# tychedelia/josefine

Measured on NVIDIA H100. Metric: Raft-group ticks/sec @ 64Ki groups x 5 replicas, higher is better.
Workload: dtype u64

## Files before the change

josefine_b200/csrc/sym_fold.cuh:

```cuda
#pragma once
#include "raft_device.cuh"

namespace jr {
#ifdef JR_DEVICE_CODE

struct SymMail {
  uint32_t hb, hb_commit;
  uint32_t ae, ae_nb, ae_id[JR_MAX_AE_BLOCKS];
  uint32_t mk;
  uint32_t hbr, hbr_commit, hbr_has;
  uint32_t ar, ar_head;
  __device__ __forceinline__ uint32_t id(uint32_t k) const {
    uint32_t v = ae_id[0];
#pragma unroll
    for (uint32_t j = 1; j < JR_MAX_AE_BLOCKS; ++j)
      if (k == j) v = ae_id[j];
    return v;
  }
  __device__ __forceinline__ void set_id(uint32_t k, uint32_t v) {
#pragma unroll
    for (uint32_t j = 0; j < JR_MAX_AE_BLOCKS; ++j)
      if (k == j) ae_id[j] = v;
  }
};

constexpr uint32_t SYM_ROWS = 8;
#ifndef JR_SYM_LANES
#define JR_SYM_LANES 128
#endif
constexpr uint32_t SYM_LANES = JR_SYM_LANES;
constexpr uint32_t SYM_ENC_L = 5, SYM_ENC_F = 3;
constexpr uint32_t SYM_SMEM_UNITS = 2 * SYM_ROWS + SYM_ENC_L + SYM_ENC_F;
constexpr uint32_t SYM2_GROUPS = 64;
constexpr uint32_t SYM2_UNITS = SYM_SMEM_UNITS + 2 * 2 + 2 * 1;
constexpr uint32_t SYM2_ABORT = 1u << 8, SYM2_IDS = 1u << 9, SYM2_MODE = 1u << 10;
enum : uint32_t {
  SP_MAIL_IN = 0,
  SP_AR = 1,
  SP_CLIENT = 2,
  SP_ENC_NOTIFY = 3,
  SP_ENC_APPLY = 4,
  SP_MAIL_OUT = 5,
  SP_BARRIER = 6,
  SP_HB = 7,
  SP_SCAN = 8,
  SP_EXTEND = 9,
  SP_ENTER = 10, SP_FILL = 11, SP_LEAVE = 12, SP_TRUNC = 13,
};

template <int R, bool SPLIT = false>
struct SymGroup {
  static constexpr uint32_t STRIDE = SPLIT ? SYM2_GROUPS : SYM_LANES;
  const Dev& d;
  const uint32_t g;
  const size_t plane;
  uint32_t L;
  uint32_t F0;
  uint64_t term, hbtime, now;
  uint32_t head, commit, idgen, maxkey, ckey, ph_self, mode_self, ph_f, mode_f;
  uint32_t fhead, fcommit, fmaxkey, fckey;
  uint32_t n_hb;
  uint64_t last_hb;
  uint32_t tbase;
  uint32_t flo;
  uint4* rows;
  uint4* enc;
  uint32_t lcnt, fcnt;
  uint32_t lwend, fwend;
  uint32_t n_app;
  bool abort;
  bool share;
#ifdef JR_PROFILE
  long long pt;
  uint32_t prole, pslot;
  __device__ __forceinline__ uint32_t phase(uint32_t slot) {
    const uint32_t o = pslot;
    if constexpr (SPLIT) {
      JR_PROF_ADD(prole, o, pt);
      pslot = slot;
    }
    return o;
  }
#else
  __device__ __forceinline__ uint32_t phase(uint32_t) const { return 0; }
#endif

  __device__ __forceinline__ SymGroup(const Dev& dv, uint32_t g_) : d(dv), g(g_), plane((size_t)R * dv.Gp) {
#ifdef JR_PROFILE
    pt = 0; prole = JR_ROLE_CANDIDATE; pslot = 0;
#endif
  }
  __device__ __forceinline__ size_t rg(uint32_t r) const { return (size_t)r * d.Gp + g; }
  __device__ __forceinline__ size_t row(uint32_t r, uint32_t bid) const { return (size_t)(bid & d.capm) * plane + rg(r); }
  __device__ __forceinline__ bool in_window(uint32_t bid) const { return bid - tbase < d.cap; }
  __device__ __forceinline__ uint4& slot(uint32_t r, uint32_t bid) const { return rows[((r == L ? 0u : SYM_ROWS) + (bid % SYM_ROWS)) * STRIDE]; }
  __device__ __forceinline__ void cache_put(uint32_t r, uint32_t bid, uint32_t nx, uint64_t tk) const {
    slot(r, bid) = make_uint4(bid, nx, (uint32_t)tk, (uint32_t)(tk >> 32));
  }
  __device__ __forceinline__ void fetch(uint32_t r, uint32_t bid, uint32_t& next, uint64_t& tok) {
    if (!in_window(bid)) { next = ABSENT; tok = 0; return; }
    const uint4 e = slot(r, bid);
    if (e.x == bid) { next = e.y; tok = (uint64_t)e.z | ((uint64_t)e.w << 32); return; }
    next = __ldcg(d.cnext + row(r, bid));
    tok = __ldcg(d.ctok + row(r, bid));
    if (!SPLIT) cache_put(r, bid, next, tok);
  }
  __device__ __forceinline__ void fetch_sent(uint32_t bid, uint32_t mk_sent, uint32_t n_app, uint32_t& next, uint64_t& tok) {
    if (!SPLIT) { fetch(L, bid, next, tok); return; }
    if (!in_window(bid)) { next = ABSENT; tok = 0; return; }
    if (bid + SYM_ROWS > mk_sent + n_app) {
      const uint4 e = slot(L, bid);
      if (e.x == bid) { next = e.y; tok = (uint64_t)e.z | ((uint64_t)e.w << 32); return; }
    }
    next = __ldcg(d.cnext + row(L, bid));
    tok = __ldcg(d.ctok + row(L, bid));
  }
  __device__ __forceinline__ void cache_clear(uint32_t first = 0, uint32_t n = 2 * SYM_ROWS) const {
#pragma unroll
    for (uint32_t k = 0; k < 2 * SYM_ROWS; ++k)
      if (k >= first && k < first + n) rows[k * STRIDE] = make_uint4(ABSENT, ABSENT, 0u, 0u);
  }
  __device__ __forceinline__ void cache_fill(uint32_t r, uint32_t top) const {
    uint32_t nx[SYM_ROWS];
    uint64_t tk[SYM_ROWS];
#pragma unroll
    for (uint32_t j = 0; j < SYM_ROWS; ++j)
      if (j <= top && in_window(top - j)) {
        nx[j] = d.cnext[row(r, top - j)];
        tk[j] = d.ctok[row(r, top - j)];
      }
#pragma unroll
    for (uint32_t j = 0; j < SYM_ROWS; ++j)
      if (j <= top && in_window(top - j)) cache_put(r, top - j, nx[j], tk[j]);
  }
  __device__ __forceinline__ bool has(uint32_t r, uint32_t bid) {
    uint32_t n; uint64_t t;
    fetch(r, bid, n, t);
    return n != ABSENT;
  }
  __device__ __forceinline__ void fetch_f(uint32_t bid, uint32_t& next, uint64_t& tok) {
    if (in_window(bid) && bid < flo) { abort = true; next = ABSENT; tok = 0; return; }
    fetch(F0, bid, next, tok);
  }
  __device__ __forceinline__ bool has_f(uint32_t bid) {
    uint32_t n; uint64_t t;
    fetch_f(bid, n, t);
    return n != ABSENT;
  }

  __device__ __forceinline__ uint4& eq(uint32_t k) const { return enc[k * STRIDE]; }
  __device__ __forceinline__ FsmOut leader_out() const { return FsmOut{d.fs + rg(L), plane, d.F, g, L}; }
  __device__ __forceinline__ FsmOut followers_out() const {
    return FsmOut{d.fs + rg(F0), plane, d.F, g, F0, ((1u << R) - 1u) & ~(1u << L)};
  }
  __device__ __forceinline__ void enc_init_leader(uint2 leader_fc) {
    eq(0) = make_uint4(leader_fc.x, leader_fc.y, leader_fc.y, 0u);
#pragma unroll
    for (uint32_t k = 1; k < SYM_ENC_L; ++k) eq(k) = make_uint4(0u, 0u, 0u, 0u);
    lwend = FS_PATTERN_BITS;
  }
  __device__ __forceinline__ void enc_init_followers() {
#pragma unroll
    for (uint32_t k = SYM_ENC_L; k < SYM_ENC_L + SYM_ENC_F; ++k) eq(k) = make_uint4(0u, 0u, 0u, 0u);
    fwend = FS_PATTERN_BITS;
  }
  template <bool NOTIFY>
  __device__ __forceinline__ bool run_extend(uint4& q, uint2& qs, uint32_t bid, uint32_t nxa, uint64_t tok) const {
    const uint4 r = q;
    if (!r.y || bid != r.x || r.y >= FS_MAX_RUN || nxa != (NOTIFY ? FSR_CLIENT : bid - 1u)) return false;
    const uint2 st = qs;
    const uint64_t step = tok - ((uint64_t)r.z | ((uint64_t)r.w << 32));
    if (r.y == 1u) {
      if (st.x != (NOTIFY ? FSR_CLIENT : bid - 2u)) return false;
      qs = make_uint2((uint32_t)step, (uint32_t)(step >> 32));
    } else if (step != ((uint64_t)st.x | ((uint64_t)st.y << 32))) {
      return false;
    }
    q = make_uint4(bid + 1u, r.y + 1u, (uint32_t)tok, (uint32_t)(tok >> 32));
    return true;
  }
  template <bool NOTIFY>
  __device__ __forceinline__ void emit_leader(uint32_t bid, uint32_t nxa, uint64_t tok) {
    if (!(d.flags & JR_F_CAPTURE_FSM)) return;
    if (lcnt >= d.Fr) { abort = true; return; }
    const uint32_t outer = phase(NOTIFY ? SP_ENC_NOTIFY : SP_ENC_APPLY);
    if (lcnt + 1u != lwend &&
        run_extend<NOTIFY>(eq(NOTIFY ? 4 : 2), reinterpret_cast<uint2*>(&eq(3))[NOTIFY ? 1 : 0], bid, nxa, tok)) {
      if (NOTIFY) {
        const uint32_t b = lcnt + FS_PATTERN_BITS - lwend;
        uint32_t* w = b < 128u ? reinterpret_cast<uint32_t*>(&eq(1)) + (b >> 5) : &eq(0).w;
        *w |= 1u << (b & 31u);
      }
      ++lcnt;
      phase(outer);
      return;
    }
    FsmEnc e;
    const uint4 q0 = eq(0);
    e.nrec = q0.x; e.seq = q0.y + lcnt; e.wseq = q0.z; e.pb2 = q0.w;
    ++lcnt;
    const bool window = NOTIFY || e.seq + 1u - e.wseq == FS_PATTERN_BITS;
    uint4 q1 = make_uint4(0u, 0u, 0u, 0u);
    if (window) q1 = eq(1);
    e.pb0 = (uint64_t)q1.x | ((uint64_t)q1.y << 32);
    e.pb1 = (uint64_t)q1.z | ((uint64_t)q1.w << 32);
    const uint4 qr = eq(NOTIFY ? 4 : 2), qs = eq(3);
    FsmRun& run = NOTIFY ? e.rn : e.ra;
    run.next_id = qr.x; run.count = qr.y;
    run.last = (uint64_t)qr.z | ((uint64_t)qr.w << 32);
    run.stride = NOTIFY ? ((uint64_t)qs.z | ((uint64_t)qs.w << 32)) : ((uint64_t)qs.x | ((uint64_t)qs.y << 32));
    fsm_enc_push<NOTIFY>(e, leader_out(), bid, nxa, tok);
    if (e.nrec != q0.x || e.wseq != q0.z || e.pb2 != q0.w) eq(0) = make_uint4(e.nrec, q0.y, e.wseq, e.pb2);
    if (window) eq(1) = make_uint4((uint32_t)e.pb0, (uint32_t)(e.pb0 >> 32), (uint32_t)e.pb1, (uint32_t)(e.pb1 >> 32));
    eq(NOTIFY ? 4 : 2) = make_uint4(run.next_id, run.count, (uint32_t)run.last, (uint32_t)(run.last >> 32));
    uint2* st = reinterpret_cast<uint2*>(&eq(3)) + (NOTIFY ? 1 : 0);
    *st = make_uint2((uint32_t)run.stride, (uint32_t)(run.stride >> 32));
    lwend = e.wseq - q0.y + FS_PATTERN_BITS;
    phase(outer);
  }
  __device__ __forceinline__ uint2 leader_end() {
    FsmEnc e;
    const uint4 q0 = eq(0), q1 = eq(1), q2 = eq(2), q3 = eq(3), q4 = eq(4);
    e.nrec = q0.x; e.seq = q0.y + lcnt; e.wseq = q0.z; e.pb2 = q0.w;
    e.pb0 = (uint64_t)q1.x | ((uint64_t)q1.y << 32);
    e.pb1 = (uint64_t)q1.z | ((uint64_t)q1.w << 32);
    e.ra = FsmRun{q2.x, q2.y, (uint64_t)q2.z | ((uint64_t)q2.w << 32), (uint64_t)q3.x | ((uint64_t)q3.y << 32)};
    e.rn = FsmRun{q4.x, q4.y, (uint64_t)q4.z | ((uint64_t)q4.w << 32), (uint64_t)q3.z | ((uint64_t)q3.w << 32)};
    return fsm_enc_end(e, leader_out());
  }
  __device__ __forceinline__ void emit_followers(uint32_t bid, uint32_t next, uint64_t tok) {
    if (!(d.flags & JR_F_CAPTURE_FSM)) return;
    if (fcnt >= d.Fr) { abort = true; return; }
    const uint32_t outer = phase(SP_ENC_APPLY);
    if (share && fcnt + 1u != fwend &&
        run_extend<false>(eq(SYM_ENC_L + 1), *reinterpret_cast<uint2*>(&eq(SYM_ENC_L + 2)), bid, next, tok)) {
    } else if (share) {
      FsmEnc e;
      const uint4 q0 = eq(SYM_ENC_L), q1 = eq(SYM_ENC_L + 1);
      const uint2 q2 = *reinterpret_cast<const uint2*>(&eq(SYM_ENC_L + 2));
      e.nrec = q0.x; e.seq = q0.y + fcnt; e.wseq = q0.z; e.pb2 = 0;
      e.pb0 = e.pb1 = 0;
      e.ra = FsmRun{q1.x, q1.y, (uint64_t)q1.z | ((uint64_t)q1.w << 32), (uint64_t)q2.x | ((uint64_t)q2.y << 32)};
      fsm_enc_push<false>(e, followers_out(), bid, next, tok);
      if (e.nrec != q0.x || e.wseq != q0.z) eq(SYM_ENC_L) = make_uint4(e.nrec, q0.y, e.wseq, 0u);
      eq(SYM_ENC_L + 1) = make_uint4(e.ra.next_id, e.ra.count, (uint32_t)e.ra.last, (uint32_t)(e.ra.last >> 32));
      *reinterpret_cast<uint2*>(&eq(SYM_ENC_L + 2)) = make_uint2((uint32_t)e.ra.stride, (uint32_t)(e.ra.stride >> 32));
      fwend = e.wseq - q0.y + FS_PATTERN_BITS;
    } else {
      const uint4 e = make_uint4(bid, next, (uint32_t)tok, (uint32_t)(tok >> 32));
#pragma unroll
      for (int r = 0; r < R; ++r)
        if ((uint32_t)r != L) d.fr[(size_t)fcnt * plane + rg(r)] = e;
    }
    ++fcnt;
    phase(outer);
  }
  __device__ __forceinline__ uint2 followers_end() {
    FsmEnc e;
    const uint4 q0 = eq(SYM_ENC_L), q1 = eq(SYM_ENC_L + 1), q2 = eq(SYM_ENC_L + 2);
    e.nrec = q0.x; e.seq = q0.y + fcnt; e.wseq = q0.z; e.pb2 = 0;
    e.pb0 = e.pb1 = 0;
    e.ra = FsmRun{q1.x, q1.y, (uint64_t)q1.z | ((uint64_t)q1.w << 32), (uint64_t)q2.x | ((uint64_t)q2.y << 32)};
    e.rn = FsmRun{0, 0, 0, 0};
    return fsm_enc_end(e, followers_out());
  }

  __device__ __forceinline__ uint32_t committed_index(uint32_t v_new, uint32_t n_new, uint32_t v_old) const {
    uint32_t v[R];
    v[0] = ph_self;
#pragma unroll
    for (int i = 1; i < R; ++i) v[i] = (uint32_t)i <= n_new ? v_new : v_old;
#pragma unroll
    for (int i = 0; i < R; ++i)
#pragma unroll
      for (int j = 0; j + 1 < R - i; ++j) {
        const uint32_t a = v[j], b = v[j + 1];
        v[j] = max(a, b);
        v[j + 1] = min(a, b);
      }
    return v[R / 2];
  }
  __device__ __forceinline__ void leader_commit(uint32_t v_new, uint32_t n_new, uint32_t v_old) {
    const uint32_t above = (ph_self > commit ? 1u : 0u) + (v_new > commit ? n_new : 0u) + (v_old > commit ? (uint32_t)(R - 1) - n_new : 0u);
    if (above < (uint32_t)(R / 2 + 1)) return;
    const uint32_t q = committed_index(v_new, n_new, v_old);
    if (q <= commit) return;
    if (!has(L, q)) { abort = true; return; }
    const uint32_t prev = commit;
    ckey = 1;
    commit = q;
    bool first = true;
    for (uint32_t b = max(prev, tbase); b <= q; ++b) {
      uint32_t nx; uint64_t tk;
      fetch(L, b, nx, tk);
      if (nx == ABSENT) continue;
      if (first) { first = false; continue; }
      emit_leader<false>(b, nx, tk);
    }
  }
  __device__ __forceinline__ void client_request(uint64_t tok) {
    const uint32_t bid = idgen++;
    if (!(bid > head) || !in_window(bid)) { abort = true; return; }
    d.cnext[row(L, bid)] = head;
    d.ctok[row(L, bid)] = tok;
    cache_put(L, bid, head, tok);
    if (bid > maxkey) maxkey = bid;
    head = bid;
    emit_leader<true>(bid, FSR_CLIENT, tok);
    mode_self = ph_self < head ? 1u : 0u;
    if (ph_self < head) ph_self = head;
    leader_commit(ph_f, R - 1, ph_f);
  }

  __device__ __forceinline__ void leader_tick(const SymMail& in, SymMail& out, uint64_t dense_tok, uint32_t n_synth,
                                              uint64_t step_index) {
    if (in.hbr && !in.hbr_has && in.hbr_commit > 0) { abort = true; return; }
    if (in.ar) {
      phase(SP_AR);
      const uint32_t old = ph_f, v = in.ar_head;
      const bool inc = old < v;
      const uint32_t nw = inc ? v : old;
      for (uint32_t j = 1; j <= (uint32_t)(R - 1) && !abort; ++j) leader_commit(nw, j, old);
      ph_f = nw;
      mode_f = inc ? 1u : 0u;
      if (abort) return;
    }
    phase(SP_CLIENT);
    if (dense_tok) client_request(dense_tok);
    for (uint32_t i = 0; i < n_synth && !abort; ++i) client_request(synth_token(step_index, i, d.goff + g));
    if (abort) return;
    phase(SP_MAIL_OUT);
    const uint64_t el = now >= hbtime ? now - hbtime : 0;
    if (el > (uint64_t)d.hb) {
      out.hb = 1;
      out.hb_commit = commit;
      hbtime = now;
    }
    out.ae = 1;
    out.mk = maxkey;
    if (!SPLIT) replicate(ph_f, mode_f, maxkey, out);
  }
  __device__ __forceinline__ void replicate(uint32_t phf, uint32_t modef, uint32_t mk, SymMail& out) {
    const uint32_t take = modef ? JR_MAX_AE_BLOCKS : 1u;
    uint32_t bid = max(phf, tbase), pulled = 0, nb = 0;
    while (pulled < 1 + take) {
      uint32_t nx = ABSENT; uint64_t tk = 0;
      while (bid <= mk) {
        fetch(L, bid, nx, tk);
        if (nx != ABSENT) break;
        ++bid;
      }
      if (bid > mk) break;
      if (pulled >= 1) out.set_id(nb++, bid);
      ++pulled;
      ++bid;
    }
    out.ae_nb = nb;
  }

  __device__ __forceinline__ void follower_heartbeat(const SymMail& in, SymMail& out) {
    phase(SP_HB);
    ++n_hb;
    last_hb = now;
    const uint32_t c = in.hb_commit;
    const bool hasc = has_f(c);
    if (hasc && c > fcommit) {
      const uint32_t prev = fcommit;
      fckey = 1;
      fcommit = c;
      for (uint32_t b = max(prev, tbase); b < c; ++b) {
        uint32_t nx; uint64_t tk;
        fetch_f(b, nx, tk);
        if (nx != ABSENT) emit_followers(b, nx, tk);
      }
    }
    out.hbr = 1;
    out.hbr_commit = fcommit;
    out.hbr_has = hasc ? 1u : 0u;
  }
  __device__ __forceinline__ void follower_extend(uint32_t bid, uint32_t nx, uint64_t tk) {
    const uint32_t outer = phase(SP_EXTEND);
    if (nx == ABSENT || !has_f(nx) || !in_window(bid)) { abort = true; return; }
#pragma unroll
    for (int r = 0; r < R; ++r)
      if ((uint32_t)r != L) {
        d.cnext[row(r, bid)] = nx;
        d.ctok[row(r, bid)] = tk;
      }
    cache_put(F0, bid, nx, tk);
    if (bid > fmaxkey) fmaxkey = bid;
    fhead = bid;
    phase(outer);
  }
  __device__ __forceinline__ void follower_tick(const SymMail& in, SymMail& out) {
    if (in.hb) follower_heartbeat(in, out);
    if (in.ae) {
      phase(SP_SCAN);
      for (uint32_t k = 0; k < in.ae_nb && !abort; ++k) {
        const uint32_t bid = in.id(k);
        uint32_t nx; uint64_t tk;
        fetch_sent(bid, in.mk, n_app, nx, tk);
        follower_extend(bid, nx, tk);
      }
      if (abort) return;
      if (in.ae_nb) {
        out.ar = 1;
        out.ar_head = fhead;
      }
    }
  }
  __device__ __forceinline__ void follower_tick_view(const SymMail& in, uint32_t phf, uint32_t modef, uint32_t mk, SymMail& out) {
    if (in.hb) follower_heartbeat(in, out);
    if (!in.ae || abort) return;
    phase(SP_SCAN);
    const uint32_t take = modef ? JR_MAX_AE_BLOCKS : 1u;
    uint32_t bid = max(phf, tbase), pulled = 0, nb = 0;
    while (pulled < 1 + take) {
      uint32_t nx = ABSENT; uint64_t tk = 0;
      while (bid <= mk) {
        fetch_sent(bid, mk, n_app, nx, tk);
        if (nx != ABSENT) break;
        ++bid;
      }
      if (bid > mk) break;
      if (pulled >= 1) {
        follower_extend(bid, nx, tk);
        if (abort) return;
        ++nb;
      }
      ++pulled;
      ++bid;
    }
    if (nb) {
      out.ar = 1;
      out.ar_head = fhead;
    }
  }
};

template <int R, bool SPLIT>
__device__ __forceinline__ bool sym_enter(SymGroup<R, SPLIT>& s, SymMail& m, const StepParams& p, int prv) {
  const Dev& d = s.d;
  if (s.g >= d.G) return false;
  uint32_t L = R, nlead = 0;
  uint4 p2[R];
#pragma unroll
  for (int r = 0; r < R; ++r) {
    p2[r] = d.p2[s.rg(r)];
    const uint32_t meta = p2[r].w;
    if (((meta >> 8) & 255u) || ((meta >> 27) & 1u)) return false;
    if ((meta & 255u) == JR_ROLE_LEADER) { L = r; ++nlead; }
    else if ((meta & 255u) != JR_ROLE_FOLLOWER) return false;
    if ((meta >> 24) & 7u) return false;
  }
  if (nlead != 1) return false;
  s.L = L;
  s.F0 = L == 0 ? 1u : 0u;
  const uint4 l0 = d.p0[s.rg(L)];
  s.term = (uint64_t)l0.x | ((uint64_t)l0.y << 32);
  s.tbase = d.tb[s.g];
  uint4 pl = p2[0], pf = p2[0];
  const uint32_t f0i = L == 0 ? 1u : 0u;
#pragma unroll
  for (int r = 0; r < R; ++r) {
    if ((uint32_t)r == L) pl = p2[r];
    if ((uint32_t)r == f0i) pf = p2[r];
  }
  s.head = pl.x; s.commit = pl.y; s.idgen = pl.z;
  s.ckey = (pl.w >> 28) & 1u;
  s.maxkey = d.mk[s.rg(L)];
  if (!(s.idgen > s.head)) return false;
  const uint4 l3 = d.p3[s.rg(L)];
  s.hbtime = (uint64_t)l3.x | ((uint64_t)l3.y << 32);
  const uint32_t f0 = s.F0;
  s.fhead = pf.x; s.fcommit = pf.y; s.fckey = (pf.w >> 28) & 1u;
  s.fmaxkey = d.mk[s.rg(f0)];
  const uint64_t hbgap = ((uint64_t)d.hb / p.dt + 1) * p.dt;
#pragma unroll
  for (int r = 0; r < R; ++r) {
    if ((uint32_t)r == L) continue;
    const uint4 a = d.p0[s.rg(r)];
    if (((uint64_t)a.x | ((uint64_t)a.y << 32)) != s.term || a.z != L + 1 || a.w != L + 1) return false;
    if (p2[r].x != s.fhead || p2[r].y != s.fcommit || ((p2[r].w >> 28) & 1u) != s.fckey) return false;
    if (d.mk[s.rg(r)] != s.fmaxkey) return false;
  }
  if ((uint64_t)d.emin <= hbgap || s.hbtime > p.now) return false;
  uint32_t ph[R];
#pragma unroll
  for (int q = 0; q < (R + 3) / 4; ++q) {
    const uint4 v = d.pr[(size_t)q * s.plane + s.rg(L)];
    if (q * 4 + 0 < R) ph[q * 4 + 0] = v.x;
    if (q * 4 + 1 < R) ph[q * 4 + 1] = v.y;
    if (q * 4 + 2 < R) ph[q * 4 + 2] = v.z;
    if (q * 4 + 3 < R) ph[q * 4 + 3] = v.w;
  }
  const uint32_t prmask = (pl.w >> 16) & 255u;
  s.ph_self = 0; s.ph_f = 0;
#pragma unroll
  for (int r = 0; r < R; ++r) {
    if ((uint32_t)r == L) s.ph_self = ph[r];
    if ((uint32_t)r == f0) s.ph_f = ph[r];
  }
  s.mode_self = (prmask >> L) & 1u;
  s.mode_f = (prmask >> f0) & 1u;
#pragma unroll
  for (int r = 0; r < R; ++r)
    if ((uint32_t)r != L && (ph[r] != s.ph_f || ((prmask >> r) & 1u) != s.mode_f)) return false;
  constexpr uint32_t SYM_WINDOW = 16;
  const uint32_t top = min(s.maxkey, s.fmaxkey);
  const uint32_t lo_min = max(top > SYM_WINDOW - 1u ? top - (SYM_WINDOW - 1u) : 0u, s.tbase);
  if (top < s.tbase || s.ph_f < lo_min || s.fcommit < lo_min || s.commit < lo_min || s.fhead < lo_min || s.fmaxkey > s.maxkey) return false;
  const uint32_t lo = min(min(s.ph_f, s.fcommit), min(s.commit, s.fhead));
  s.flo = lo;
  const uint64_t grow = (uint64_t)p.n_ticks * (1u + p.n_synth) + 2u;
  if ((uint64_t)s.maxkey + grow >= (uint64_t)s.tbase + d.cap || (uint64_t)s.maxkey + grow >= FS_NOTIFY_BIT) return false;
  {
    constexpr uint32_t B = 4;
    bool same = true;
    for (uint32_t b0 = lo; b0 <= s.fmaxkey && same; b0 += B) {
      uint32_t n0[B];
      unsigned long long t0[B];
#pragma unroll
      for (uint32_t j = 0; j < B; ++j) {
        const uint32_t b = min(b0 + j, s.fmaxkey);
        n0[j] = d.cnext[s.row(f0, b)];
        t0[j] = d.ctok[s.row(f0, b)];
      }
#pragma unroll
      for (int r = 0; r < R; ++r) {
        if ((uint32_t)r == L || (uint32_t)r == f0) continue;
#pragma unroll
        for (uint32_t j = 0; j < B; ++j) {
          const uint32_t b = min(b0 + j, s.fmaxkey);
          const uint32_t n = d.cnext[s.row(r, b)];
          const unsigned long long t = d.ctok[s.row(r, b)];
          same = same && n == n0[j] && (n0[j] == ABSENT || t == t0[j]);
        }
      }
    }
    if (!same) return false;
  }
  m = SymMail{};
  if (p.phases & PH_DRAIN) {
  {
    const uint32_t cnt = d.oc[prv][s.rg(L)];
    uint32_t u = 0;
    auto unit = [&](uint32_t k) { return d.ob[prv][((size_t)k * R + L) * d.Gp + s.g]; };
    if (cnt > (uint32_t)(1 + JR_MAX_AE_BLOCKS + R)) return false;
    if (u < cnt) {
      const uint4 h = unit(u);
      if ((h.x & 15u) == JR_CMD_HEARTBEAT) {
        if ((h.x >> 16) != TO_PEERS || ((uint64_t)h.y | ((uint64_t)h.z << 32)) != s.term) return false;
        m.hb = 1; m.hb_commit = h.w;
        ++u;
      }
    }
    if (u < cnt) {
      uint32_t first = 0;
      for (int r = 0; r < R; ++r) {
        if ((uint32_t)r == L) continue;
        if (u >= cnt) return false;
        const uint4 h = unit(u);
        if ((h.x & 15u) != JR_CMD_APPEND_ENTRIES || (h.x >> 16) != (uint32_t)r + 1u ||
            ((uint64_t)h.y | ((uint64_t)h.z << 32)) != s.term) return false;
        const uint32_t nb = (h.x >> 8) & 255u, ref = (h.x >> 4) & 1u;
        if (!m.ae) {
          if (ref || nb > JR_MAX_AE_BLOCKS || h.w != u + 1 || u + 1 + nb > cnt) return false;
          m.ae = 1; m.ae_nb = nb; first = u + 1;
          for (uint32_t k = 0; k < nb; ++k) {
            const uint4 bu = unit(first + k);
            uint32_t nx; uint64_t tk;
            s.fetch(L, bu.x, nx, tk);
            if (nx != bu.y || tk != ((uint64_t)bu.z | ((uint64_t)bu.w << 32))) return false;
            m.set_id(k, bu.x);
          }
          u += 1 + nb;
        } else {
          if (!ref || nb != m.ae_nb || h.w != first) return false;
          ++u;
        }
      }
    }
    if (u != cnt) return false;
  }
  {
    const uint32_t cnt = d.oc[prv][s.rg(f0)];
    if (cnt > 2) return false;
    uint4 want[2] = {make_uint4(0, 0, 0, 0), make_uint4(0, 0, 0, 0)};
    for (uint32_t u = 0; u < cnt; ++u) want[u] = d.ob[prv][((size_t)u * R + f0) * d.Gp + s.g];
#pragma unroll
    for (int r = 0; r < R; ++r) {
      if ((uint32_t)r == L || (uint32_t)r == f0) continue;
      if (d.oc[prv][s.rg(r)] != cnt) return false;
      for (uint32_t u = 0; u < cnt; ++u) {
        const uint4 v = d.ob[prv][((size_t)u * R + r) * d.Gp + s.g];
        if (v.x != want[u].x || v.y != want[u].y || v.z != want[u].z || v.w != want[u].w) return false;
      }
    }
    uint32_t u = 0;
    if (u < cnt && (want[u].x & 15u) == JR_CMD_HEARTBEAT_RESPONSE) {
      if ((want[u].x >> 16) != L + 1) return false;
      m.hbr = 1; m.hbr_has = (want[u].x >> 4) & 1u; m.hbr_commit = want[u].w;
      ++u;
    }
    if (u < cnt && (want[u].x & 15u) == JR_CMD_APPEND_RESPONSE) {
      if ((want[u].x >> 16) != L + 1 || ((uint64_t)want[u].y | ((uint64_t)want[u].z << 32)) != s.term) return false;
      m.ar = 1; m.ar_head = want[u].w;
      ++u;
    }
    if (u != cnt) return false;
  }
  }
  uint64_t t_arr = 0;
  if (!m.hb) {
    const uint64_t due = s.hbtime + (uint64_t)d.hb + 1;
    t_arr = (due > p.now ? (due - p.now + p.dt - 1) / p.dt : 0) + 1;
  }
  const uint64_t checked = t_arr < p.n_ticks ? t_arr : p.n_ticks;
  if (checked) {
    const uint64_t t_last = p.now + (checked - 1) * p.dt;
#pragma unroll
    for (int r = 0; r < R; ++r) {
      if ((uint32_t)r == L) continue;
      const uint4 b = d.p1[s.rg(r)];
      const uint64_t etime = (uint64_t)b.x | ((uint64_t)b.y << 32);
      if (t_last >= etime && t_last - etime > (uint64_t)b.z) return false;
    }
  }
  return true;
}

template <int R, bool SPLIT>
__device__ __forceinline__ void sym_leave_leader(SymGroup<R, SPLIT>& s, const SymMail& last, int cur_last) {
  const Dev& d = s.d;
  const uint32_t L = s.L;
  {
    const size_t i = s.rg(L);
    uint32_t prmask = 0;
#pragma unroll
    for (int r = 0; r < R; ++r) prmask |= (((uint32_t)r == L ? s.mode_self : s.mode_f) & 1u) << r;
    const uint32_t keep = d.p2[i].w & ~((255u << 16) | (1u << 28));
    d.p2[i] = make_uint4(s.head, s.commit, s.idgen, keep | (prmask << 16) | (s.ckey << 28));
    d.p3[i] = make_uint4((uint32_t)s.hbtime, (uint32_t)(s.hbtime >> 32), 0u, 0u);
#pragma unroll
    for (int q = 0; q < (R + 3) / 4; ++q) {
      uint32_t v[4] = {0, 0, 0, 0};
#pragma unroll
      for (int k = 0; k < 4; ++k)
        if (q * 4 + k < R) v[k] = (uint32_t)(q * 4 + k) == L ? s.ph_self : s.ph_f;
      d.pr[(size_t)q * s.plane + i] = make_uint4(v[0], v[1], v[2], v[3]);
    }
    d.mk[i] = s.maxkey;
    uint32_t u = 0;
    auto put = [&](uint32_t k, uint4 v) { d.ob[cur_last][((size_t)k * R + L) * d.Gp + s.g] = v; };
    if (last.hb) put(u++, make_uint4(unit_hdr(JR_CMD_HEARTBEAT, 0, 0, TO_PEERS), (uint32_t)s.term, (uint32_t)(s.term >> 32), last.hb_commit));
    if (last.ae) {
      uint32_t first = 0;
      bool have = false;
#pragma unroll
      for (int r = 0; r < R; ++r) {
        if ((uint32_t)r == L) continue;
        if (!have) {
          first = u + 1;
          put(u, make_uint4(unit_hdr(JR_CMD_APPEND_ENTRIES, 0, last.ae_nb, r + 1), (uint32_t)s.term, (uint32_t)(s.term >> 32), first));
          for (uint32_t k = 0; k < last.ae_nb; ++k) {
            const uint32_t bid = last.id(k);
            uint32_t nx; uint64_t tk;
            s.fetch(L, bid, nx, tk);
            put(first + k, make_uint4(bid, nx, (uint32_t)tk, (uint32_t)(tk >> 32)));
          }
          u += 1 + last.ae_nb;
          have = true;
        } else {
          put(u++, make_uint4(unit_hdr(JR_CMD_APPEND_ENTRIES, 1, last.ae_nb, r + 1), (uint32_t)s.term, (uint32_t)(s.term >> 32), first));
        }
      }
    }
    d.oc[cur_last][i] = u;
    if ((d.flags & JR_F_CAPTURE_FSM) && s.lcnt) d.fc[i] = s.leader_end();
  }
}

template <int R, bool SPLIT>
__device__ __forceinline__ void sym_leave_followers(SymGroup<R, SPLIT>& s, const SymMail& last, int cur_last) {
  const Dev& d = s.d;
  const uint32_t L = s.L;
  const bool shared_records = s.share;
#pragma unroll
  for (int r = 0; r < R; ++r) {
    if ((uint32_t)r == L) continue;
    const size_t i = s.rg(r);
    if (s.n_hb) {
      const uint4 b = d.p1[i];
      const uint32_t draws = b.w + s.n_hb;
      d.p1[i] = make_uint4((uint32_t)s.last_hb, (uint32_t)(s.last_hb >> 32),
                           election_timeout_draw(d.seed, d.goff + s.g, r + 1, draws - 1, d.emin, d.emax), draws);
    }
    const uint4 c = d.p2[i];
    d.p2[i] = make_uint4(s.fhead, s.fcommit, c.z, (c.w & ~(1u << 28)) | (s.fckey << 28));
    d.mk[i] = s.fmaxkey;
    uint32_t u = 0;
    if (last.hbr)
      d.ob[cur_last][((size_t)u++ * R + r) * d.Gp + s.g] =
          make_uint4(unit_hdr(JR_CMD_HEARTBEAT_RESPONSE, last.hbr_has, 0, L + 1), 0u, 0u, last.hbr_commit);
    if (last.ar)
      d.ob[cur_last][((size_t)u++ * R + r) * d.Gp + s.g] =
          make_uint4(unit_hdr(JR_CMD_APPEND_RESPONSE, 1, 0, L + 1), (uint32_t)s.term, (uint32_t)(s.term >> 32), last.ar_head);
    d.oc[cur_last][i] = u;
    if ((d.flags & JR_F_CAPTURE_FSM) && s.fcnt) {
      if (!shared_records) fsm_flush(d.fr + i, s.fcnt, d.Fr, FsmOut{d.fs + i, s.plane, d.F, s.g, (uint32_t)r}, d.fc + i);
      else if ((uint32_t)r == s.F0) d.fc[i] = s.followers_end();
      else d.fc[i] = make_uint2(0u, s.fcnt);
    }
  }
}

template <int R>
__global__ void __launch_bounds__(SYM_LANES, 512 / SYM_LANES) sym_kernel(const Dev d, const StepParams p, uint8_t* symdone) {
  const uint32_t g = blockIdx.x * blockDim.x + threadIdx.x;
  if (g >= d.Gp) return;
  SymGroup<R> s(d, g);
  SymMail a, b;
  s.abort = false;
  s.lcnt = s.fcnt = 0;
  s.n_hb = 0;
  s.last_hb = 0;
  s.share = false;
  s.n_app = 1u + p.n_synth;
  __shared__ uint4 lane_smem[SYM_SMEM_UNITS * SYM_LANES];
  s.rows = lane_smem + threadIdx.x;
  s.enc = lane_smem + 2 * SYM_ROWS * SYM_LANES + threadIdx.x;
  s.cache_clear();
  bool ok = sym_enter(s, a, p, 1 - p.cur);
  if (ok) {
    s.cache_fill(s.L, s.maxkey);
    s.cache_fill(s.F0, s.fmaxkey);
    s.share = (d.flags & JR_F_CAPTURE_FSM) != 0;
#pragma unroll
    for (int r = 0; r < R; ++r) {
      if ((uint32_t)r == s.L) continue;
      const uint2 c = d.fc[s.rg(r)];
      if (c.x | c.y) s.share = false;
    }
    s.enc_init_leader((d.flags & JR_F_CAPTURE_FSM) ? d.fc[s.rg(s.L)] : make_uint2(0u, 0u));
    s.enc_init_followers();
    const jr_proposal* props = p.proposals;
    s.now = p.now;
    for (uint32_t t = 0; t < p.n_ticks && !s.abort; ++t) {
      b = SymMail{};
      uint64_t tok = 0;
      if ((p.phases & PH_PROPOSE) && (props || p.tok_runs)) {
        uint4 pr;
        if (p.tok_runs) {
          const uint4 rn = __ldg(p.tok_runs + g);
          const uint64_t base = (uint64_t)rn.x | ((uint64_t)rn.y << 32);
          const uint64_t tk = base + (uint64_t)(p.tok_tick + t) * ((uint64_t)rn.z | ((uint64_t)rn.w << 32));
          pr = make_uint4((uint32_t)tk, (uint32_t)(tk >> 32), base ? __ldg(p.tok_route + g) : 0u, 0u);
        } else {
          pr = __ldg(reinterpret_cast<const uint4*>(props) + g);
          props += p.prop_stride;
        }
        if (pr.z == s.L + 1) tok = (uint64_t)pr.x | ((uint64_t)pr.y << 32);
        else if (pr.z != 0) s.abort = true;
      }
      if (s.abort) break;
      s.leader_tick(a, b, tok, (p.phases & PH_PROPOSE) ? p.n_synth : 0u, p.step_index + t);
      if (s.abort) break;
      s.follower_tick(a, b);
      a = b;
      s.now += p.dt;
    }
    ok = !s.abort;
    if (ok) {
      const int cur_last = p.cur ^ (int)((p.n_ticks - 1) & 1u);
      sym_leave_leader(s, a, cur_last);
      sym_leave_followers(s, a, cur_last);
    }
  }
  symdone[g] = ok ? 1 : 0;
}

#ifndef JR_SYM2_MINCTAS
#define JR_SYM2_MINCTAS 4
#endif
#ifndef JR_SYM2_ROLES
#define JR_SYM2_ROLES 3
#endif
template <int R>
__global__ void __launch_bounds__(2 * SYM2_GROUPS, JR_SYM2_MINCTAS) sym2_kernel(const Dev d, const StepParams p, uint8_t* symdone, uint8_t* symblk) {
  JR_DYN_SMEM(uint4, smem);
  auto pair_sync = [] { __syncthreads(); };
  constexpr uint32_t S = SYM2_GROUPS;
  const uint32_t w = threadIdx.x >> 5, lane = threadIdx.x & 31u;
  const bool lead = ((w ^ blockIdx.x) & 1u) == 0;
  const uint32_t gi = (w >> 1) * 32u + lane;
  const uint32_t g = blockIdx.x * S + gi;
  SymGroup<R, true> s(d, g);
  s.abort = false;
  s.lcnt = s.fcnt = 0;
  s.n_hb = 0;
  s.last_hb = 0;
  s.share = false;
  s.n_app = 1u + p.n_synth;
  s.rows = smem + gi;
  s.enc = smem + 2 * SYM_ROWS * S + gi;
  uint4* mail = smem + SYM_SMEM_UNITS * S + gi;
#ifdef JR_PROFILE
  for (uint32_t i = threadIdx.x; i < 8 * 3 * 16 * 2; i += blockDim.x) jr_prof_smem()[i] = 0;
  s.prole = lead ? JR_ROLE_LEADER : JR_ROLE_FOLLOWER;
  s.pslot = SP_ENTER;
  s.pt = clock64();
#endif
  s.cache_clear(lead ? 0u : SYM_ROWS, SYM_ROWS);
  const uint32_t blk = g / GROUPS_PER_CTA;
  if (lead && lane == 0 && g < d.Gp) symblk[blk] = 1;
  pair_sync();
  SymMail a;
  bool dead = !sym_enter(s, a, p, 1 - p.cur);
  pair_sync();
  s.phase(SP_FILL);
  if (!dead) {
    if (lead) {
      s.cache_fill(s.L, s.maxkey);
      s.enc_init_leader((d.flags & JR_F_CAPTURE_FSM) ? d.fc[s.rg(s.L)] : make_uint2(0u, 0u));
      mail[2 * S] = make_uint4(a.hb | (a.ae << 1) | (a.ae_nb << 4) | SYM2_IDS, a.hb_commit, s.maxkey, a.ae_id[0]);
      mail[3 * S] = make_uint4(a.ae_id[1], a.ae_id[2], a.ae_id[3], a.ae_id[4]);
    } else {
      s.cache_fill(s.F0, s.fmaxkey);
      s.enc_init_followers();
      s.share = (d.flags & JR_F_CAPTURE_FSM) != 0;
#pragma unroll
      for (int r = 0; r < R; ++r) {
        if ((uint32_t)r == s.L) continue;
        const uint2 c = d.fc[s.rg(r)];
        if (c.x | c.y) s.share = false;
      }
      mail[5 * S] = make_uint4(a.hbr | (a.hbr_has << 1) | (a.ar << 2), a.hbr_commit, a.ar_head, 0u);
    }
  }
  pair_sync();
  const jr_proposal* props = p.proposals;
  s.now = p.now;
  uint32_t cur = 0;
  for (uint32_t t = 0; t < p.n_ticks; ++t) {
    s.phase(SP_MAIL_IN);
    if (lead && (JR_SYM2_ROLES & 1)) {
      if (!dead) {
        const uint4 c = mail[(4 + (1 - cur)) * S];
        if (c.x & SYM2_ABORT) dead = true;
        else {
          SymMail in{}, out{};
          in.hbr = c.x & 1u; in.hbr_has = (c.x >> 1) & 1u; in.ar = (c.x >> 2) & 1u;
          in.hbr_commit = c.y; in.ar_head = c.z;
          uint64_t tok = 0;
          if ((p.phases & PH_PROPOSE) && (props || p.tok_runs)) {
            uint4 pr;
            if (p.tok_runs) {
              const uint4 rn = __ldg(p.tok_runs + g);
              const uint64_t base = (uint64_t)rn.x | ((uint64_t)rn.y << 32);
              const uint64_t tk = base + (uint64_t)(p.tok_tick + t) * ((uint64_t)rn.z | ((uint64_t)rn.w << 32));
              pr = make_uint4((uint32_t)tk, (uint32_t)(tk >> 32), base ? __ldg(p.tok_route + g) : 0u, 0u);
            } else {
              pr = __ldg(reinterpret_cast<const uint4*>(props + (size_t)t * p.prop_stride) + g);
            }
            if (pr.z == s.L + 1) tok = (uint64_t)pr.x | ((uint64_t)pr.y << 32);
            else if (pr.z != 0) s.abort = true;
          }
          if (!s.abort) s.leader_tick(in, out, tok, (p.phases & PH_PROPOSE) ? p.n_synth : 0u, p.step_index + t);
          if (s.abort) dead = true;
          else {
            mail[(2 * cur) * S] = make_uint4(out.hb | (out.ae << 1) | (s.mode_f ? SYM2_MODE : 0u), s.commit, s.maxkey, s.ph_f);
          }
        }
      }
      if (dead) mail[(2 * cur) * S] = make_uint4(SYM2_ABORT, 0u, 0u, 0u);
    } else if (!lead && (JR_SYM2_ROLES & 2)) {
      if (!dead) {
        const uint4 ma = mail[(2 * (1 - cur)) * S];
        if (ma.x & SYM2_ABORT) dead = true;
        else {
          SymMail in{}, out{};
          in.hb = ma.x & 1u; in.ae = (ma.x >> 1) & 1u;
          in.hb_commit = ma.y; in.mk = ma.z;
          if (ma.x & SYM2_IDS) {
            const uint4 mb = mail[(2 * (1 - cur) + 1) * S];
            in.ae_nb = (ma.x >> 4) & 15u;
            in.ae_id[0] = ma.w; in.ae_id[1] = mb.x; in.ae_id[2] = mb.y; in.ae_id[3] = mb.z; in.ae_id[4] = mb.w;
            s.follower_tick(in, out);
          } else {
            s.follower_tick_view(in, ma.w, (ma.x & SYM2_MODE) ? 1u : 0u, ma.z, out);
          }
          s.phase(SP_MAIL_OUT);
          if (s.abort) dead = true;
          else mail[(4 + cur) * S] = make_uint4(out.hbr | (out.hbr_has << 1) | (out.ar << 2), out.hbr_commit, out.ar_head, 0u);
        }
      }
      if (dead) mail[(4 + cur) * S] = make_uint4(SYM2_ABORT, 0u, 0u, 0u);
    }
    s.now += p.dt;
    s.phase(SP_BARRIER);
    pair_sync();
    cur ^= 1u;
  }
  s.phase(SP_LEAVE);
  const uint32_t lastb = cur ^ 1u;
  const uint4 la = mail[(2 * lastb) * S], lc = mail[(4 + lastb) * S];
  const bool ok = !dead && !((la.x | lc.x) & SYM2_ABORT);
  if (ok) {
    const int cur_last = p.cur ^ (int)((p.n_ticks - 1) & 1u);
    SymMail last{};
    if (lead) {
      last.hb = la.x & 1u; last.ae = (la.x >> 1) & 1u;
      last.hb_commit = la.y;
      if (last.ae) s.replicate(s.ph_f, s.mode_f, s.maxkey, last);
      sym_leave_leader(s, last, cur_last);
    } else {
      last.hbr = lc.x & 1u; last.hbr_has = (lc.x >> 1) & 1u; last.ar = (lc.x >> 2) & 1u;
      last.hbr_commit = lc.y; last.ar_head = lc.z;
      sym_leave_followers(s, last, cur_last);
    }
  }
  s.phase(SP_TRUNC);
  if (p.trunc) {
    pair_sync();
    if (ok && !lead) {
      const uint32_t lo = min(s.fcommit, la.y);
      const uint32_t floor = lo > p.trunc_margin ? lo - p.trunc_margin : 0u;
      if (floor > s.tbase) {
        for (uint32_t b = s.tbase; b < floor && b - s.tbase < d.cap; ++b)
#pragma unroll
          for (int r = 0; r < R; ++r) d.cnext[s.row(r, b)] = ABSENT;
        d.tb[g] = floor;
      }
    }
  }
  if (lead && g < d.Gp) {
    symdone[g] = ok ? 1 : 0;
    if (!ok) {
      symblk[blk] = 0;
      if (g < d.G) *(volatile uint32_t*)d.hunf = p.epoch;
    }
  }
#ifdef JR_PROFILE
  s.phase(SP_TRUNC);
  __syncthreads();
  if (d.prof)
    for (uint32_t i = threadIdx.x; i < 4 * 3 * 16 * 2; i += blockDim.x) {
      const unsigned long long v = jr_prof_smem()[i];
      if (v) atomicAdd(d.prof + (i % (3 * 16 * 2)), v);
    }
#endif
}

__global__ void sym_blocks_kernel(const uint8_t* symdone, uint8_t* symblk, uint32_t n_blocks) {
  const uint32_t b = blockIdx.x * blockDim.x + threadIdx.x;
  if (b >= n_blocks) return;
  const uint4* v = reinterpret_cast<const uint4*>(symdone + (size_t)b * GROUPS_PER_CTA);
  const uint4 x = v[0], y = v[1];
  const uint32_t all = 0x01010101u;
  symblk[b] = (x.x == all && x.y == all && x.z == all && x.w == all && y.x == all && y.y == all && y.z == all && y.w == all) ? 1 : 0;
}

#endif
}
```

Measured before the change: 11.14 billion.

## Split symmetric-fold entry check into leader and follower sides with batched loads

Turns sym_enter into a side-templated check so that, in the paired kernel, the leader thread validates its outbox while the follower thread validates follower state, mailbox agreement and election timers. The two verdicts are exchanged through shared memory and combined. Global loads (p2, mk, oc, outbox units, vote and timer state) are hoisted and issued together rather than interleaved with early returns, and the cache fills move into the entry check. The aim is to halve the serial entry latency per pair and raise memory-level parallelism, at the cost of more registers and extra loads that can no longer be skipped by an early exit. The single-thread path now calls both sides in sequence.

```diff
diff --git a/josefine_b200/csrc/sym_fold.cuh b/josefine_b200/csrc/sym_fold.cuh
--- a/josefine_b200/csrc/sym_fold.cuh
+++ b/josefine_b200/csrc/sym_fold.cuh
@@ -70,6 +70,7 @@
   uint32_t n_app;
   bool abort;
   bool share;
+  uint2 lfc;
 #ifdef JR_PROFILE
   long long pt;
   uint32_t prole, pslot;
@@ -438,85 +439,214 @@
   }
 };
 
-template <int R, bool SPLIT>
-__device__ __forceinline__ bool sym_enter(SymGroup<R, SPLIT>& s, SymMail& m, const StepParams& p, int prv) {
+constexpr uint32_t SYM_SIDE_LEADER = 1, SYM_SIDE_FOLLOWERS = 2;
+constexpr int SYM_FCHUNK = 5;
+constexpr uint32_t SYM_OK = 1,
+                   SYM_TIMER_OK = 2,
+                   SYM_HB = 4;
+__device__ __forceinline__ bool sym_accept(uint32_t vl, uint32_t vf) {
+  return (vl & vf & SYM_OK) && ((vl & SYM_HB) || (vf & SYM_TIMER_OK));
+}
+
+template <uint32_t SIDE, int R, bool SPLIT>
+__device__ __forceinline__ uint32_t sym_enter(SymGroup<R, SPLIT>& s, SymMail& m, const StepParams& p, int prv) {
   const Dev& d = s.d;
-  if (s.g >= d.G) return false;
-  uint32_t L = R, nlead = 0;
+  if (s.g >= d.G) return 0;
+  constexpr bool lside = SIDE == SYM_SIDE_LEADER, fside = SIDE == SYM_SIDE_FOLLOWERS;
+  const bool drain = (p.phases & PH_DRAIN) != 0;
+  const bool capture = (d.flags & JR_F_CAPTURE_FSM) != 0;
   uint4 p2[R];
+  uint32_t mk[R], oc[R];
 #pragma unroll
   for (int r = 0; r < R; ++r) {
     p2[r] = d.p2[s.rg(r)];
+    mk[r] = d.mk[s.rg(r)];
+    oc[r] = drain ? d.oc[prv][s.rg(r)] : 0u;
+  }
+  s.tbase = d.tb[s.g];
+  uint32_t L = R, nlead = 0;
+  bool ok = true;
+#pragma unroll
+  for (int r = 0; r < R; ++r) {
     const uint32_t meta = p2[r].w;
-    if (((meta >> 8) & 255u) || ((meta >> 27) & 1u)) return false;
+    if (((meta >> 8) & 255u) || ((meta >> 27) & 1u)) ok = false;
     if ((meta & 255u) == JR_ROLE_LEADER) { L = r; ++nlead; }
-    else if ((meta & 255u) != JR_ROLE_FOLLOWER) return false;
-    if ((meta >> 24) & 7u) return false;
-  }
-  if (nlead != 1) return false;
+    else if ((meta & 255u) != JR_ROLE_FOLLOWER) ok = false;
+    if ((meta >> 24) & 7u) ok = false;
+  }
+  if (!ok || nlead != 1) return 0;
+  const uint32_t f0 = L == 0 ? 1u : 0u;
   s.L = L;
-  s.F0 = L == 0 ? 1u : 0u;
-  const uint4 l0 = d.p0[s.rg(L)];
-  s.term = (uint64_t)l0.x | ((uint64_t)l0.y << 32);
-  s.tbase = d.tb[s.g];
+  s.F0 = f0;
   uint4 pl = p2[0], pf = p2[0];
-  const uint32_t f0i = L == 0 ? 1u : 0u;
+  uint32_t ocl = oc[0], ocf = oc[0];
+  s.maxkey = mk[0]; s.fmaxkey = mk[0];
 #pragma unroll
   for (int r = 0; r < R; ++r) {
-    if ((uint32_t)r == L) pl = p2[r];
-    if ((uint32_t)r == f0i) pf = p2[r];
+    if ((uint32_t)r == L) { pl = p2[r]; s.maxkey = mk[r]; ocl = oc[r]; }
+    if ((uint32_t)r == f0) { pf = p2[r]; s.fmaxkey = mk[r]; ocf = oc[r]; }
   }
   s.head = pl.x; s.commit = pl.y; s.idgen = pl.z;
   s.ckey = (pl.w >> 28) & 1u;
-  s.maxkey = d.mk[s.rg(L)];
-  if (!(s.idgen > s.head)) return false;
+  if (!(s.idgen > s.head)) return 0;
+  s.fhead = pf.x; s.fcommit = pf.y; s.fckey = (pf.w >> 28) & 1u;
+#pragma unroll
+  for (int r = 0; r < R; ++r)
+    if ((uint32_t)r != L && (p2[r].x != s.fhead || p2[r].y != s.fcommit || ((p2[r].w >> 28) & 1u) != s.fckey || mk[r] != s.fmaxkey))
+      return 0;
+  const uint4 l0 = d.p0[s.rg(L)];
   const uint4 l3 = d.p3[s.rg(L)];
+  uint4 prq[(R + 3) / 4];
+#pragma unroll
+  for (int q = 0; q < (R + 3) / 4; ++q) prq[q] = d.pr[(size_t)q * s.plane + s.rg(L)];
+  constexpr uint32_t NU = R + JR_MAX_AE_BLOCKS;
+  uint4 lu[NU];
+  const uint32_t nu = min(min(ocl, d.U), NU);
+  uint4 fp0[R], fp1[R];
+  uint32_t fcs = 0;
+  if constexpr (lside) {
+#pragma unroll
+    for (uint32_t k = 0; k < NU; ++k)
+      lu[k] = k < nu ? d.ob[prv][((size_t)k * R + L) * d.Gp + s.g] : make_uint4(0u, 0u, 0u, 0u);
+    s.lfc = capture ? d.fc[s.rg(L)] : make_uint2(0u, 0u);
+  }
+  if constexpr (fside) {
+#pragma unroll
+    for (int r = 0; r < R; ++r) {
+      if ((uint32_t)r == L) continue;
+      if (r < SYM_FCHUNK) {
+        fp0[r] = d.p0[s.rg(r)];
+        fp1[r] = d.p1[s.rg(r)];
+      }
+      const uint2 c = d.fc[s.rg(r)];
+      fcs |= c.x | c.y;
+    }
+  }
+  s.term = (uint64_t)l0.x | ((uint64_t)l0.y << 32);
   s.hbtime = (uint64_t)l3.x | ((uint64_t)l3.y << 32);
-  const uint32_t f0 = s.F0;
-  s.fhead = pf.x; s.fcommit = pf.y; s.fckey = (pf.w >> 28) & 1u;
-  s.fmaxkey = d.mk[s.rg(f0)];
   const uint64_t hbgap = ((uint64_t)d.hb / p.dt + 1) * p.dt;
-#pragma unroll
-  for (int r = 0; r < R; ++r) {
-    if ((uint32_t)r == L) continue;
-    const uint4 a = d.p0[s.rg(r)];
-    if (((uint64_t)a.x | ((uint64_t)a.y << 32)) != s.term || a.z != L + 1 || a.w != L + 1) return false;
-    if (p2[r].x != s.fhead || p2[r].y != s.fcommit || ((p2[r].w >> 28) & 1u) != s.fckey) return false;
-    if (d.mk[s.rg(r)] != s.fmaxkey) return false;
-  }
-  if ((uint64_t)d.emin <= hbgap || s.hbtime > p.now) return false;
-  uint32_t ph[R];
-#pragma unroll
-  for (int q = 0; q < (R + 3) / 4; ++q) {
-    const uint4 v = d.pr[(size_t)q * s.plane + s.rg(L)];
-    if (q * 4 + 0 < R) ph[q * 4 + 0] = v.x;
-    if (q * 4 + 1 < R) ph[q * 4 + 1] = v.y;
-    if (q * 4 + 2 < R) ph[q * 4 + 2] = v.z;
-    if (q * 4 + 3 < R) ph[q * 4 + 3] = v.w;
-  }
+  if ((uint64_t)d.emin <= hbgap || s.hbtime > p.now) return 0;
   const uint32_t prmask = (pl.w >> 16) & 255u;
   s.ph_self = 0; s.ph_f = 0;
 #pragma unroll
   for (int r = 0; r < R; ++r) {
-    if ((uint32_t)r == L) s.ph_self = ph[r];
-    if ((uint32_t)r == f0) s.ph_f = ph[r];
+    const uint4 v = prq[r / 4];
+    const uint32_t ph = (r & 3) == 0 ? v.x : (r & 3) == 1 ? v.y : (r & 3) == 2 ? v.z : v.w;
+    if ((uint32_t)r == L) s.ph_self = ph;
+    if ((uint32_t)r == f0) s.ph_f = ph;
   }
   s.mode_self = (prmask >> L) & 1u;
   s.mode_f = (prmask >> f0) & 1u;
 #pragma unroll
-  for (int r = 0; r < R; ++r)
-    if ((uint32_t)r != L && (ph[r] != s.ph_f || ((prmask >> r) & 1u) != s.mode_f)) return false;
+  for (int r = 0; r < R; ++r) {
+    const uint4 v = prq[r / 4];
+    const uint32_t ph = (r & 3) == 0 ? v.x : (r & 3) == 1 ? v.y : (r & 3) == 2 ? v.z : v.w;
+    if ((uint32_t)r != L && (ph != s.ph_f || ((prmask >> r) & 1u) != s.mode_f)) return 0;
+  }
   constexpr uint32_t SYM_WINDOW = 16;
   const uint32_t top = min(s.maxkey, s.fmaxkey);
   const uint32_t lo_min = max(top > SYM_WINDOW - 1u ? top - (SYM_WINDOW - 1u) : 0u, s.tbase);
-  if (top < s.tbase || s.ph_f < lo_min || s.fcommit < lo_min || s.commit < lo_min || s.fhead < lo_min || s.fmaxkey > s.maxkey) return false;
+  if (top < s.tbase || s.ph_f < lo_min || s.fcommit < lo_min || s.commit < lo_min || s.fhead < lo_min || s.fmaxkey > s.maxkey) return 0;
   const uint32_t lo = min(min(s.ph_f, s.fcommit), min(s.commit, s.fhead));
   s.flo = lo;
   const uint64_t grow = (uint64_t)p.n_ticks * (1u + p.n_synth) + 2u;
-  if ((uint64_t)s.maxkey + grow >= (uint64_t)s.tbase + d.cap || (uint64_t)s.maxkey + grow >= FS_NOTIFY_BIT) return false;
-  {
+  if ((uint64_t)s.maxkey + grow >= (uint64_t)s.tbase + d.cap || (uint64_t)s.maxkey + grow >= FS_NOTIFY_BIT) return 0;
+  uint32_t verdict = SYM_OK;
+  if constexpr (lside) {
+    s.cache_fill(L, s.maxkey);
+    if (ocl) {
+      const bool hb = (lu[0].x & 15u) == JR_CMD_HEARTBEAT;
+      const uint32_t u0 = hb ? 1u : 0u;
+      if (hb) {
+        if ((lu[0].x >> 16) != TO_PEERS || lu[0].y != l0.x || lu[0].z != l0.y) return 0;
+        m.hb = 1; m.hb_commit = lu[0].w;
+      }
+      if (ocl > u0) {
+        const uint4 h = hb ? lu[1] : lu[0];
+        const uint32_t nb = (h.x >> 8) & 255u;
+        if ((h.x & 15u) != JR_CMD_APPEND_ENTRIES || (h.x >> 16) != f0 + 1u || h.y != l0.x || h.z != l0.y ||
+            ((h.x >> 4) & 1u) || nb > JR_MAX_AE_BLOCKS || h.w != u0 + 1u || ocl != u0 + 1u + nb + (uint32_t)(R - 2)) return 0;
+        m.ae = 1; m.ae_nb = nb;
+        bool same = true;
+#pragma unroll
+        for (uint32_t k = 1; k < NU; ++k) {
+          const uint4 v = lu[k];
+          if (k > u0 && k <= u0 + nb) {
+            uint32_t nx; uint64_t tk;
+            s.fetch(L, v.x, nx, tk);
+            same = same && nx == v.y && tk == ((uint64_t)v.z | ((uint64_t)v.w << 32));
+            m.set_id(k - u0 - 1u, v.x);
+          } else if (k > u0 + nb && k < ocl) {
+            const uint32_t j = k - u0 - nb, r = j + (j >= L ? 1u : 0u);
+            same = same && (v.x & 15u) == JR_CMD_APPEND_ENTRIES && (v.x >> 16) == r + 1u && v.y == l0.x && v.z == l0.y &&
+                   ((v.x >> 4) & 1u) && ((v.x >> 8) & 255u) == nb && v.w == u0 + 1u;
+          }
+        }
+        if (!same) return 0;
+      }
+    }
+    if (m.hb) verdict |= SYM_HB;
+  }
+  if constexpr (fside) {
+    s.share = capture && !fcs;
+    uint64_t t_last = 0;
+    {
+      const uint64_t due = s.hbtime + (uint64_t)d.hb + 1;
+      const uint64_t t_arr = (due > p.now ? (due - p.now + p.dt - 1) / p.dt : 0) + 1;
+      const uint64_t checked = t_arr < p.n_ticks ? t_arr : p.n_ticks;
+      t_last = checked ? p.now + (checked - 1) * p.dt : 0;
+      bool timers = true, votes = true;
+#pragma unroll
+      for (int r = 0; r < R; ++r) {
+        if ((uint32_t)r == L) continue;
+        const uint4 a = r < SYM_FCHUNK ? fp0[r] : d.p0[s.rg(r)], b = r < SYM_FCHUNK ? fp1[r] : d.p1[s.rg(r)];
+        votes = votes && ((uint64_t)a.x | ((uint64_t)a.y << 32)) == s.term && a.z == L + 1 && a.w == L + 1;
+        const uint64_t etime = (uint64_t)b.x | ((uint64_t)b.y << 32);
+        if (checked && t_last >= etime && t_last - etime > (uint64_t)b.z) timers = false;
+      }
+      if (!votes) return 0;
+      if (timers) verdict |= SYM_TIMER_OK;
+    }
+    if (ocf > 2) return 0;
+    s.cache_fill(f0, s.fmaxkey);
+    uint4 fu[R][2];
+    const uint32_t nfu = min(ocf, d.U);
+#pragma unroll
+    for (int r = 0; r < R && r < SYM_FCHUNK; ++r) {
+      if ((uint32_t)r == L) continue;
+#pragma unroll
+      for (uint32_t u = 0; u < 2; ++u)
+        fu[r][u] = u < nfu ? d.ob[prv][((size_t)u * R + r) * d.Gp + s.g] : make_uint4(0u, 0u, 0u, 0u);
+    }
+    bool same = true;
+    uint4 w0 = fu[0][0], w1 = fu[0][1];
+#pragma unroll
+    for (int r = 0; r < 2; ++r)
+      if ((uint32_t)r == f0) { w0 = fu[r][0]; w1 = fu[r][1]; }
+#pragma unroll
+    for (int r = 0; r < R; ++r) {
+      if ((uint32_t)r == L || (uint32_t)r == f0) continue;
+      const uint4 z = make_uint4(0u, 0u, 0u, 0u);
+      const uint4 v0 = r < SYM_FCHUNK ? fu[r][0] : 0u < nfu ? d.ob[prv][(size_t)r * d.Gp + s.g] : z;
+      const uint4 v1 = r < SYM_FCHUNK ? fu[r][1] : 1u < nfu ? d.ob[prv][((size_t)R + r) * d.Gp + s.g] : z;
+      same = same && oc[r] == ocf && (ocf < 1 || (v0.x == w0.x && v0.y == w0.y && v0.z == w0.z && v0.w == w0.w)) &&
+             (ocf < 2 || (v1.x == w1.x && v1.y == w1.y && v1.z == w1.z && v1.w == w1.w));
+    }
+    if (!same) return 0;
+    uint32_t u = 0;
+    if (u < ocf && (w0.x & 15u) == JR_CMD_HEARTBEAT_RESPONSE) {
+      if ((w0.x >> 16) != L + 1) return 0;
+      m.hbr = 1; m.hbr_has = (w0.x >> 4) & 1u; m.hbr_commit = w0.w;
+      ++u;
+    }
+    const uint4 w = u ? w1 : w0;
+    if (u < ocf && (w.x & 15u) == JR_CMD_APPEND_RESPONSE) {
+      if ((w.x >> 16) != L + 1 || w.y != l0.x || w.z != l0.y) return 0;
+      m.ar = 1; m.ar_head = w.w;
+      ++u;
+    }
+    if (u != ocf) return 0;
     constexpr uint32_t B = 4;
-    bool same = true;
     for (uint32_t b0 = lo; b0 <= s.fmaxkey && same; b0 += B) {
       uint32_t n0[B];
       unsigned long long t0[B];
@@ -538,96 +668,9 @@
         }
       }
     }
-    if (!same) return false;
-  }
-  m = SymMail{};
-  if (p.phases & PH_DRAIN) {
-  {
-    const uint32_t cnt = d.oc[prv][s.rg(L)];
-    uint32_t u = 0;
-    auto unit = [&](uint32_t k) { return d.ob[prv][((size_t)k * R + L) * d.Gp + s.g]; };
-    if (cnt > (uint32_t)(1 + JR_MAX_AE_BLOCKS + R)) return false;
-    if (u < cnt) {
-      const uint4 h = unit(u);
-      if ((h.x & 15u) == JR_CMD_HEARTBEAT) {
-        if ((h.x >> 16) != TO_PEERS || ((uint64_t)h.y | ((uint64_t)h.z << 32)) != s.term) return false;
-        m.hb = 1; m.hb_commit = h.w;
-        ++u;
-      }
-    }
-    if (u < cnt) {
-      uint32_t first = 0;
-      for (int r = 0; r < R; ++r) {
-        if ((uint32_t)r == L) continue;
-        if (u >= cnt) return false;
-        const uint4 h = unit(u);
-        if ((h.x & 15u) != JR_CMD_APPEND_ENTRIES || (h.x >> 16) != (uint32_t)r + 1u ||
-            ((uint64_t)h.y | ((uint64_t)h.z << 32)) != s.term) return false;
-        const uint32_t nb = (h.x >> 8) & 255u, ref = (h.x >> 4) & 1u;
-        if (!m.ae) {
-          if (ref || nb > JR_MAX_AE_BLOCKS || h.w != u + 1 || u + 1 + nb > cnt) return false;
-          m.ae = 1; m.ae_nb = nb; first = u + 1;
-          for (uint32_t k = 0; k < nb; ++k) {
-            const uint4 bu = unit(first + k);
-            uint32_t nx; uint64_t tk;
-            s.fetch(L, bu.x, nx, tk);
-            if (nx != bu.y || tk != ((uint64_t)bu.z | ((uint64_t)bu.w << 32))) return false;
-            m.set_id(k, bu.x);
-          }
-          u += 1 + nb;
-        } else {
-          if (!ref || nb != m.ae_nb || h.w != first) return false;
-          ++u;
-        }
-      }
-    }
-    if (u != cnt) return false;
-  }
-  {
-    const uint32_t cnt = d.oc[prv][s.rg(f0)];
-    if (cnt > 2) return false;
-    uint4 want[2] = {make_uint4(0, 0, 0, 0), make_uint4(0, 0, 0, 0)};
-    for (uint32_t u = 0; u < cnt; ++u) want[u] = d.ob[prv][((size_t)u * R + f0) * d.Gp + s.g];
-#pragma unroll
-    for (int r = 0; r < R; ++r) {
-      if ((uint32_t)r == L || (uint32_t)r == f0) continue;
-      if (d.oc[prv][s.rg(r)] != cnt) return false;
-      for (uint32_t u = 0; u < cnt; ++u) {
-        const uint4 v = d.ob[prv][((size_t)u * R + r) * d.Gp + s.g];
-        if (v.x != want[u].x || v.y != want[u].y || v.z != want[u].z || v.w != want[u].w) return false;
-      }
-    }
-    uint32_t u = 0;
-    if (u < cnt && (want[u].x & 15u) == JR_CMD_HEARTBEAT_RESPONSE) {
-      if ((want[u].x >> 16) != L + 1) return false;
-      m.hbr = 1; m.hbr_has = (want[u].x >> 4) & 1u; m.hbr_commit = want[u].w;
-      ++u;
-    }
-    if (u < cnt && (want[u].x & 15u) == JR_CMD_APPEND_RESPONSE) {
-      if ((want[u].x >> 16) != L + 1 || ((uint64_t)want[u].y | ((uint64_t)want[u].z << 32)) != s.term) return false;
-      m.ar = 1; m.ar_head = want[u].w;
-      ++u;
-    }
-    if (u != cnt) return false;
-  }
-  }
-  uint64_t t_arr = 0;
-  if (!m.hb) {
-    const uint64_t due = s.hbtime + (uint64_t)d.hb + 1;
-    t_arr = (due > p.now ? (due - p.now + p.dt - 1) / p.dt : 0) + 1;
-  }
-  const uint64_t checked = t_arr < p.n_ticks ? t_arr : p.n_ticks;
-  if (checked) {
-    const uint64_t t_last = p.now + (checked - 1) * p.dt;
-#pragma unroll
-    for (int r = 0; r < R; ++r) {
-      if ((uint32_t)r == L) continue;
-      const uint4 b = d.p1[s.rg(r)];
-      const uint64_t etime = (uint64_t)b.x | ((uint64_t)b.y << 32);
-      if (t_last >= etime && t_last - etime > (uint64_t)b.z) return false;
-    }
-  }
-  return true;
+    if (!same) return 0;
+  }
+  return verdict;
 }
 
 template <int R, bool SPLIT>
@@ -720,7 +763,7 @@
   const uint32_t g = blockIdx.x * blockDim.x + threadIdx.x;
   if (g >= d.Gp) return;
   SymGroup<R> s(d, g);
-  SymMail a, b;
+  SymMail a{}, b;
   s.abort = false;
   s.lcnt = s.fcnt = 0;
   s.n_hb = 0;
@@ -731,18 +774,10 @@
   s.rows = lane_smem + threadIdx.x;
   s.enc = lane_smem + 2 * SYM_ROWS * SYM_LANES + threadIdx.x;
   s.cache_clear();
-  bool ok = sym_enter(s, a, p, 1 - p.cur);
+  const uint32_t vl = sym_enter<SYM_SIDE_LEADER>(s, a, p, 1 - p.cur);
+  bool ok = sym_accept(vl, vl & SYM_OK ? sym_enter<SYM_SIDE_FOLLOWERS>(s, a, p, 1 - p.cur) : 0u);
   if (ok) {
-    s.cache_fill(s.L, s.maxkey);
-    s.cache_fill(s.F0, s.fmaxkey);
-    s.share = (d.flags & JR_F_CAPTURE_FSM) != 0;
-#pragma unroll
-    for (int r = 0; r < R; ++r) {
-      if ((uint32_t)r == s.L) continue;
-      const uint2 c = d.fc[s.rg(r)];
-      if (c.x | c.y) s.share = false;
-    }
-    s.enc_init_leader((d.flags & JR_F_CAPTURE_FSM) ? d.fc[s.rg(s.L)] : make_uint2(0u, 0u));
+    s.enc_init_leader(s.lfc);
     s.enc_init_followers();
     const jr_proposal* props = p.proposals;
     s.now = p.now;
@@ -815,26 +850,20 @@
   const uint32_t blk = g / GROUPS_PER_CTA;
   if (lead && lane == 0 && g < d.Gp) symblk[blk] = 1;
   pair_sync();
-  SymMail a;
-  bool dead = !sym_enter(s, a, p, 1 - p.cur);
+  SymMail a{};
+  const uint32_t v = lead ? sym_enter<SYM_SIDE_LEADER>(s, a, p, 1 - p.cur) : sym_enter<SYM_SIDE_FOLLOWERS>(s, a, p, 1 - p.cur);
+  mail[(lead ? 0 : 4) * S] = make_uint4(v, 0u, 0u, 0u);
   pair_sync();
+  const uint32_t vo = mail[(lead ? 4 : 0) * S].x;
+  bool dead = !(lead ? sym_accept(v, vo) : sym_accept(vo, v));
   s.phase(SP_FILL);
   if (!dead) {
     if (lead) {
-      s.cache_fill(s.L, s.maxkey);
-      s.enc_init_leader((d.flags & JR_F_CAPTURE_FSM) ? d.fc[s.rg(s.L)] : make_uint2(0u, 0u));
+      s.enc_init_leader(s.lfc);
       mail[2 * S] = make_uint4(a.hb | (a.ae << 1) | (a.ae_nb << 4) | SYM2_IDS, a.hb_commit, s.maxkey, a.ae_id[0]);
       mail[3 * S] = make_uint4(a.ae_id[1], a.ae_id[2], a.ae_id[3], a.ae_id[4]);
     } else {
-      s.cache_fill(s.F0, s.fmaxkey);
       s.enc_init_followers();
-      s.share = (d.flags & JR_F_CAPTURE_FSM) != 0;
-#pragma unroll
-      for (int r = 0; r < R; ++r) {
-        if ((uint32_t)r == s.L) continue;
-        const uint2 c = d.fc[s.rg(r)];
-        if (c.x | c.y) s.share = false;
-      }
       mail[5 * S] = make_uint4(a.hbr | (a.hbr_has << 1) | (a.ar << 2), a.hbr_commit, a.ar_head, 0u);
     }
   }
```

Measured after the change: 11.92 billion, median of 6. +7.0%, better.
